# SonyCSLParis/audio-metrics

Measured on AMD Instinct MI355X. Metric: evaluate() embeddings/sec (FAD+KD+PRDC), 2×100k CLAP-512 sets, 1/2/4/8 GPUs, higher is better.
Workload: dtype f32

## Files before the change

audio-metrics_amd/csrc/pairwise.hip:

```cpp
#include "pairwise_common.h"
#include <algorithm>
#include <vector>
#include <cmath>
#include <type_traits>

namespace am {

__global__ void __launch_bounds__(256) row_sqnorm_kernel(const float* __restrict__ X, int64_t N, int64_t ld,
                                                         int D, float* __restrict__ out) {
    const int lane = threadIdx.x & 63;
    const int64_t row = (int64_t)blockIdx.x * 4 + (threadIdx.x >> 6);
    if (row >= N) return;
    const float* x = X + row * ld;
    float acc = 0.f;
    for (int k = lane * 4; k < D; k += 256) {
        const f32x4 v = load_k4(x, k, D);
        acc = fmaf(v.x, v.x, acc);
        acc = fmaf(v.y, v.y, acc);
        acc = fmaf(v.z, v.z, acc);
        acc = fmaf(v.w, v.w, acc);
    }
#pragma unroll
    for (int off = 32; off >= 1; off >>= 1) acc = acc + __shfl_xor(acc, off);
    if (lane == 0) out[row] = acc;
}

__device__ __forceinline__ float threshold_of_radius(float R) {
    if (!(R > 0.f)) return 0.f;
    if (isinf(R)) return R;
    float c = R * R;
    for (int it = 0; it < 8; ++it) {
        const float p = __uint_as_float(__float_as_uint(c) - 1u);
        if (c > 0.f && sqrt_rn(p) >= R) c = p; else break;
    }
    for (int it = 0; it < 8; ++it) {
        if (sqrt_rn(c) < R) c = __uint_as_float(__float_as_uint(c) + 1u); else break;
    }
    return c;
}

__global__ void threshold_kernel(const float* __restrict__ R, int64_t n, float* __restrict__ T) {
    const int64_t i = (int64_t)blockIdx.x * blockDim.x + threadIdx.x;
    if (i < n) T[i] = threshold_of_radius(R[i]);
}

struct DenseRows {
    const float* base;
    int64_t ld, n, tile0;
    __device__ __forceinline__ const float* operator()(int t, int row) const {
        const int64_t g = (tile0 + t) * TB + row;
        return g < n ? base + g * ld : nullptr;
    }
};

static inline int64_t cross_grouped_blocks(int64_t row_blocks, int nchunks, int grp_rows) {
    const int grp_chunks = 64 / grp_rows;
    const int64_t groups = ceil_div(row_blocks, grp_rows) * ceil_div(nchunks, grp_chunks);
// ... 1211 lines not shown
    hipLaunchKernelGGL(narrow64_kernel, dim3((unsigned)ceil_div(Nr, 256)), dim3(256), 0, st, rt, Nr, L.rt);
    hipLaunchKernelGGL(narrow64_kernel, dim3((unsigned)ceil_div(Nc, 256)), dim3(256), 0, st, ct, Nc, L.ct);
    hipLaunchKernelGGL(fill_u32_kernel, dim3((unsigned)ceil_div(Nr, 256)), dim3(256), 0, st, L.rmin, Nr, 0x7f800000u);
    AM_LAUNCH_CHECK();
    int rc;
    if ((rc = norms_of(nullptr, L.r32, Nr, L.ld32, D, L.rn, st)) != AM_OK) return rc;
    if ((rc = norms_of(nullptr, L.c32, Nc, L.ld32, D, L.cn, st)) != AM_OK) return rc;
    const Prdc64Hook h{R, C, ldr, ldc, rt, ct};
    if ((rc = run_cross_fast(L.r32, Nr, L.ld32, L.rn, L.rt, L.c32, Nc, L.ld32, L.cn, L.ct, D, L.plan, L.buf, col_count, L.rmin, row_any,
                             row_cover, false, st, nullptr, nullptr, &h)) != AM_OK)
        return rc;
    *fail_flag = L.buf.ov_count + 1;
    return AM_OK;
}

}

extern "C" int am_knn_radii_f32(const float* X, int64_t N, int64_t ldx, const float* Y, int64_t M, int64_t ldy,
                                int D, int k, float* out_r, void* ws, size_t ws_bytes, am_stream_t stream) {
    return knn_radii_impl(X, N, ldx, Y, M, ldy, D, k, out_r, ws, ws_bytes, stream, nullptr);
}

static bool prepared_ok(const am_prepared_set* p) { return p != nullptr && p->norms != nullptr && p->stats != nullptr && p->half != nullptr; }
static PreparedSet prepared_of(const am_prepared_set* p) { return PreparedSet{p->norms, p->stats, p->half}; }

extern "C" int64_t am_prepared_half_ld(int D) { return D < 1 ? 0 : half_ld(D); }

extern "C" int am_prepare_set_f32(const float* X, int64_t N, int64_t ld, int D, float* norms, uint32_t* stats4, uint16_t* half,
                                  am_stream_t stream) {
    int rc;
    if ((rc = check_matrix(X, N, ld, D, "X")) != AM_OK) return rc;
    AM_REQUIRE(norms && stats4 && half, AM_ERR_BAD_ARG, "null output pointer");
    hipStream_t st = static_cast<hipStream_t>(stream);
    if ((rc = launch_norms(X, N, ld, D, norms, st)) != AM_OK) return rc;
    AM_HIP_TRY(hipMemsetAsync(stats4, 0, 4 * sizeof(unsigned), st));
    return launch_to_half(X, N, ld, D, norms, stats4, 0, half, st);
}

extern "C" int am_knn_radii_prepared_f32(const float* X, int64_t N, int64_t ldx, int D, const am_prepared_set* prepared, int k,
                                         float* out_r, void* ws, size_t ws_bytes, am_stream_t stream) {
    AM_REQUIRE(prepared_ok(prepared), AM_ERR_BAD_ARG, "prepared set has a null member");
    const PreparedSet ps = prepared_of(prepared);
    return knn_radii_impl(X, N, ldx, X, N, ldx, D, k, out_r, ws, ws_bytes, stream, &ps);
}

extern "C" int am_filter_stats_enable(int64_t* device_slots) {
    if (device_slots == nullptr) {
        g_filter_stats = nullptr;
        g_filter_stats_device = -1;
        return AM_OK;
    }
    int dev = -1;
    AM_HIP_TRY(hipGetDevice(&dev));
    g_filter_stats = reinterpret_cast<long long*>(device_slots);
    g_filter_stats_device = dev;
    return AM_OK;
}

extern "C" int am_knn_path(int64_t N, int64_t M, int D, int k, int self) {
    if (N < 1 || M < 1 || D < 1 || k < 1) return -1;
    if (k > AM_MAX_K) return 4;
    const KnnPlan p = plan_knn(N, M, D, k, self != 0 && N == M);
    return !p.sym ? 0 : (knn_fast_enabled(N, D) ? (p.tile_rows == 256 ? 3 : 2) : 1);
}
extern "C" int am_prdc_path(int64_t Nr, int64_t Nc, int D) {
    if (Nr < 1 || Nc < 1 || D < 1) return -1;
    if (!cross_fast_enabled(Nr, Nc, D)) return 0;
    return plan_cross_fast(Nr, Nc, D).wide ? 3 : 2;
}
// ... 333 lines not shown
```

audio-metrics_amd/csrc/pairwise_fast.h:

```cpp
#pragma once

namespace am {

constexpr int EV_FAST = EV_DEFAULT | EV_F16 | EV_LDS;
constexpr int FAST_MAX_DIM = 4096;
constexpr int FAST_MIN_DIM = 1;
constexpr int FAST_DROP_BITS = 0;
static inline int half_drop_bits() {
    static const int n = std::min(std::max(env_int("AM_HALF_DROP_BITS", FAST_DROP_BITS), 0), 6);
    return n;
}
static inline float fast_c(int D) {
    const int n = half_drop_bits();
    const float rest = 1.9073486328125e-06f + 2.98023223876953125e-08f * sqrtf((float)D) + (float)(D + 1) * 4.76837158203125e-07f;
    if (n == 0) return 0.0009765625f + rest;
    const float u = ldexpf(1.f, -(11 - n)) + ldexpf(1.f, -11);
    return 2.f * u + u * u + rest;
}
constexpr int FAST_LDH_ALIGN = 64;

static inline int64_t half_ld(int D) { return (int64_t)(D + FAST_LDH_ALIGN - 1) / FAST_LDH_ALIGN * FAST_LDH_ALIGN; }

__global__ void __launch_bounds__(256) maxabs_bits_kernel(const float* __restrict__ X, int64_t N, int64_t ld, int D,
                                                          unsigned* __restrict__ out) {
// ... 56 lines not shown
static long long* g_filter_stats = nullptr;
static int g_filter_stats_device = -1;

static long long* filter_stats_for_current_device() {
    if (g_filter_stats == nullptr) return nullptr;
    int dev = -1;
    if (hipGetDevice(&dev) != hipSuccess || dev != g_filter_stats_device) return nullptr;
    return g_filter_stats;
}

__global__ void __launch_bounds__(256) filter_stats_kernel(const int* __restrict__ wgq_count, int64_t nwg, long long* __restrict__ stats,
                                                           int slot_calls, int slot_queued, const unsigned long long* spill64,
                                                           const int* spill32, int spill_cap, int slot_spill, const int* extra_a,
                                                           int slot_a, const int* extra_b, int slot_b) {
    long long q = 0;
    for (int64_t i = threadIdx.x; i < nwg; i += 256) q += wgq_count[i];
#pragma unroll
    for (int off = 32; off >= 1; off >>= 1) q += __shfl_xor(q, off);
    __shared__ long long red[4];
    if ((threadIdx.x & 63) == 0) red[threadIdx.x >> 6] = q;
    __syncthreads();
    if (threadIdx.x == 0) {
        long long spill = 0;
        if (spill64 != nullptr) spill = (long long)min(*spill64, (unsigned long long)spill_cap);
        if (spill32 != nullptr) spill = min(*spill32, spill_cap);
        atomicAdd(reinterpret_cast<unsigned long long*>(stats + slot_calls), 1ull);
        atomicAdd(reinterpret_cast<unsigned long long*>(stats + slot_queued), (unsigned long long)(red[0] + red[1] + red[2] + red[3] + spill));
        atomicAdd(reinterpret_cast<unsigned long long*>(stats + slot_spill), (unsigned long long)spill);
        if (extra_a != nullptr) atomicAdd(reinterpret_cast<unsigned long long*>(stats + slot_a), (unsigned long long)*extra_a);
        if (extra_b != nullptr) atomicAdd(reinterpret_cast<unsigned long long*>(stats + slot_b), (unsigned long long)*extra_b);
    }
}

static int launch_to_half(const float* X, int64_t N, int64_t ld, int D, const float* norms, unsigned* stats, int which,
                          uint16_t* Xh, hipStream_t st) {
    const int64_t ldh = half_ld(D);
    hipLaunchKernelGGL(max_bits_kernel, dim3(256), dim3(256), 0, st, norms, N, stats + which);
    hipLaunchKernelGGL(maxabs_bits_kernel, dim3((unsigned)std::min<int64_t>(ceil_div(N, 4), 1024)), dim3(256), 0, st, X, N, ld, D,
                       stats + 2 + which);
    const int64_t threads = N * (ldh / 8);
    hipLaunchKernelGGL(to_half_kernel, dim3((unsigned)ceil_div(threads, 256)), dim3(256), 0, st, X, N, ld, D, ldh,
                       stats + 2 + which, Xh, half_drop_bits());
    AM_LAUNCH_CHECK();
    return AM_OK;
}

struct PreparedSet {
    const float* norms;
    const unsigned* stats;
    const uint16_t* half;
};

__global__ void prepared_stats_kernel(const unsigned* __restrict__ stats, unsigned* __restrict__ maxn, int slot_norm, int slot_abs,
                                      int slot_abs2) {
    if (threadIdx.x == 0) {
        maxn[slot_norm] = stats[0];
        maxn[slot_abs] = stats[2];
        if (slot_abs2 >= 0) maxn[slot_abs2] = stats[2];
    }
}

static int norms_of(const PreparedSet* prep, const float* X, int64_t N, int64_t ld, int D, float* out, hipStream_t st) {
    if (prep != nullptr) {
        AM_HIP_TRY(hipMemcpyAsync(out, prep->norms, (size_t)N * sizeof(float), hipMemcpyDeviceToDevice, st));
        return AM_OK;
    }
    return launch_norms(X, N, ld, D, out, st);
}

__device__ __forceinline__ float exact_pair_dot(const float* __restrict__ xs, const float* __restrict__ y, int D) {
    float acc = 0.f;
    const int dp = (D + 7) / 8 * 8;
    for (int c = 0; c < dp; c += 8) {
        const f32x4 y0 = load_k4(y, c, D), y1 = load_k4(y, c + 4, D);
        const f32x4 x0 = *reinterpret_cast<const f32x4*>(xs + c), x1 = *reinterpret_cast<const f32x4*>(xs + c + 4);
#pragma unroll
        for (int s = 0; s < 4; ++s) {
            acc = fmaf(y0[s], x0[s], acc);
            acc = fmaf(y1[s], x1[s], acc);
        }
    }
    return acc;
}

constexpr int FAST_AUX_FLOATS = 6 * TB;
constexpr size_t FAST_LDS_BYTES = (ENGINE_LDS_FLOATS + FAST_AUX_FLOATS) * sizeof(float) + 16;

struct CrossFastEpilogue {
    const float* qnorm;
    const float* qthr;
    int64_t nq;
    float fc;
// ... 519 lines not shown
};

static CrossFastBuffers carve_cross_fast(Carver& c, int64_t Nr, int64_t Nc, int D, const CrossFastPlan& p) {
    CrossFastBuffers b;
    b.rb = c.take<uint16_t>((size_t)Nr * half_ld(D));
    b.cb = c.take<uint16_t>((size_t)Nc * half_ld(D));
    b.maxn = c.take<unsigned>(4);
    b.rmin_approx = c.take<unsigned>(Nr);
    b.wgq = c.take<uint2>((size_t)p.blocks * p.qcap);
    b.ovq = c.take<uint2>((size_t)p.ovcap);
    b.items = c.take<uint2>((size_t)p.blocks * ((p.qcap + 63) / 64));
    b.wgq_count = c.take<int>(p.blocks);
    b.ov_count = c.take<int>(4);
    return b;
}

static bool cross_fast_enabled(int64_t Nr, int64_t Nc, int D) {
    static const int on = env_int("AM_PRDC_FAST", 1);
    static const int min_pairs_env = env_int("AM_FAST_MIN_PAIRS_LOG2", 0);
    const int64_t min_pairs_n = min_pairs_env > 0 ? ((int64_t)1 << min_pairs_env)
                                                  : (D >= 256 ? (int64_t)1 << 24 : D >= 128 ? (int64_t)1 << 26 : D >= 32 ? (int64_t)100000000 : (int64_t)1 << 28);
    const size_t verify_lds = (size_t)(4 * ((D + 7) / 8 * 8) + 2048) * sizeof(float);
    return on != 0 && D >= FAST_MIN_DIM && D <= FAST_MAX_DIM && verify_lds <= 60 * 1024 && Nr * Nc >= min_pairs_n &&
           Nr < ((int64_t)1 << 31) && Nc < ((int64_t)1 << 31);
}

static int run_cross_fast(const float* R, int64_t Nr, int64_t ldr, const float* rn, const float* rt, const float* C, int64_t Nc,
                          int64_t ldc, const float* cn, const float* ct, int D, const CrossFastPlan& p, const CrossFastBuffers& b,
                          int32_t* col_count, unsigned* rmin, unsigned* rany, unsigned* rcov, bool want_min, hipStream_t st,
                          const PreparedSet* prep_r = nullptr, const PreparedSet* prep_c = nullptr, const Prdc64Hook* h64 = nullptr) {
    int rc;
    const float fc = h64 != nullptr ? fast_c(D) + 3.814697265625e-06f : fast_c(D);
    AM_REQUIRE(h64 == nullptr || (p.wide && !want_min), AM_ERR_BAD_ARG, "the float64 route is the 256-row form without row minima");
    AM_HIP_TRY(hipMemsetAsync(b.maxn, 0, 4 * sizeof(unsigned), st));
    AM_HIP_TRY(hipMemsetAsync(b.ov_count, 0, 4 * sizeof(int), st));
    if (prep_r != nullptr) hipLaunchKernelGGL(prepared_stats_kernel, dim3(1), dim3(64), 0, st, prep_r->stats, b.maxn, 0, 2, -1);
    else if ((rc = launch_to_half(R, Nr, ldr, D, rn, b.maxn, 0, b.rb, st)) != AM_OK) return rc;
    if (prep_c != nullptr) hipLaunchKernelGGL(prepared_stats_kernel, dim3(1), dim3(64), 0, st, prep_c->stats, b.maxn, 1, 3, -1);
    else if ((rc = launch_to_half(C, Nc, ldc, D, cn, b.maxn, 1, b.cb, st)) != AM_OK) return rc;
    hipLaunchKernelGGL(fill_u32_kernel, dim3((unsigned)ceil_div(Nr, 256)), dim3(256), 0, st, b.rmin_approx, Nr, 0x7f800000u);
    AM_LAUNCH_CHECK();
    const int64_t ldb = half_ld(D);
    const int Dh = (int)(ldb / 2);
    const float* Rb = reinterpret_cast<const float*>(prep_r != nullptr ? prep_r->half : b.rb);
    const float* Cb = reinterpret_cast<const float*>(prep_c != nullptr ? prep_c->half : b.cb);
    int* fail = b.ov_count + 1;
    {
        const void* kernels[] = {reinterpret_cast<const void*>(&cross_fast_kernel<true, true>),
                                 reinterpret_cast<const void*>(&cross_fast_kernel<true, false>),
                                 reinterpret_cast<const void*>(&cross_fast_kernel<false, true>),
                                 reinterpret_cast<const void*>(&cross_fast_kernel<false, false>)};
        for (const void* k : kernels)
            AM_HIP_TRY(ensure_dynamic_lds(k, (int)FAST_LDS_BYTES));
    }
    const int dbg = env_int("AM_FAST_DBG", 0);
    auto launch_filter = [&](auto kernel, unsigned grid, int nchunks, int qstride, int grp_rows) {
        hipLaunchKernelGGL(kernel, dim3(grid), dim3(ENGINE_THREADS), FAST_LDS_BYTES, st, Rb, Nr, ldb / 2, rn, rt, Cb, Nc, ldb / 2,
                           cn, ct, Dh, nchunks, qstride, b.maxn, b.rmin_approx, rany, rcov, col_count, b.wgq, p.qcap, b.wgq_count,
                           b.ovq, b.ov_count, p.ovcap, fail, dbg, fc, grp_rows);
    };
    const unsigned pre_grid = (unsigned)(ceil_div(Nr, TB) * p.pre_chunks);
    static const int pre_any = env_int("AM_FAST_PRE_ANY", 1);
    if (want_min) launch_filter(&cross_fast_kernel<true, true>, pre_grid, p.pre_chunks, p.qstride, 0);
    else if (pre_any == 1 && p.wide) {
        const int64_t samples = ceil_div(ceil_div(Nc, WIDE_TILE_ROWS), p.qstride), rbs = ceil_div(Nr, WIDE_TILE_ROWS);
        int chunks = 1;
        int64_t best_cost = INT64_MAX;
        for (int c = 1; c <= 12 && c <= samples; ++c) {
            const int64_t cost = ceil_div(rbs * c, 256) * (ceil_div(samples, c) + 1);
            if (cost < best_cost) {
                best_cost = cost;
                chunks = c;
            }
// ... 162 lines not shown
                for (int s = 0; s < KCAP; ++s)
                    if (v[s] > -INFINITY) list_insert<KCAP>(m, v[s]);
            }
            float* out = partial + ((int64_t)sw.W * N + i) * KCAP;
#pragma unroll
            for (int s = 0; s < KCAP; ++s) __hip_atomic_store(out + s, m[s], __ATOMIC_RELAXED, __HIP_MEMORY_SCOPE_AGENT);
            const float kthv = m[KCAP - 1];
            const float bound = kthv + 2.f * fc * (xnorm[i] + nmax);
            if (epi_row_in_sweep(thr, i)) atomicMin(reinterpret_cast<unsigned*>(thr) + i, __float_as_uint(bound));
        }
    }
}

__global__ void __launch_bounds__(256) knn_fast_bound_kernel(const float* __restrict__ in, float* __restrict__ thr,
                                                             const float* __restrict__ xnorm, int64_t n,
                                                             const unsigned* __restrict__ maxn, float factor ) {
    const int64_t i = (int64_t)blockIdx.x * 256 + threadIdx.x;
    if (i < n) thr[i] = in[i] + factor * (xnorm[i] + __uint_as_float(maxn[0]));
}

__device__ __forceinline__ void knn_file_approx(float* __restrict__ fval, unsigned* __restrict__ fidx, int* __restrict__ cnt,
                                                int cap, int64_t row, float v, unsigned partner) {
    const int slot = atomicAdd(cnt + row, 1);
    if (slot < cap) {
        fval[row * (int64_t)cap + slot] = v;
        fidx[row * (int64_t)cap + slot] = partner;
    }
}

__global__ void __launch_bounds__(256) knn_fast_scatter_kernel(const uint2* __restrict__ wgq, const float* __restrict__ wgv,
                                                               int qcap, int wcap, int nsub, const int* __restrict__ wgq_count,
                                                               float* __restrict__ fval, unsigned* __restrict__ fidx,
                                                               int* __restrict__ cnt, int cap, const float* __restrict__ thr,
                                                               const int* __restrict__ skip) {
    if (skip != nullptr && *skip != 0) return;
    const int n = wgq_count[blockIdx.x];
    const int64_t base = (int64_t)(blockIdx.x / (nsub + 1)) * qcap + (int64_t)(blockIdx.x % (nsub + 1)) * wcap;
    const uint2* q = wgq + base;
    const float* v = wgv + base;
    for (int e = threadIdx.x; e < n; e += 256) {
        const uint2 p = q[e];
        const unsigned a = p.x & ~FAST_BOTH;
        const float val = v[e];
        if (val <= thr[a]) knn_file_approx(fval, fidx, cnt, cap, a, val, p.y);
        if ((p.x & FAST_BOTH) && val <= thr[p.y]) knn_file_approx(fval, fidx, cnt, cap, p.y, val, a);
    }
}

__global__ void __launch_bounds__(256) knn_fast_scatter_spill_kernel(const uint2* __restrict__ ovq, const float* __restrict__ ovv,
                                                                     const unsigned long long* __restrict__ ovn, int ovcap,
                                                                     float* __restrict__ fval, unsigned* __restrict__ fidx,
                                                                     int* __restrict__ cnt, int cap, const float* __restrict__ thr,
                                                                     const int* __restrict__ skip) {
    if (skip != nullptr && *skip != 0) return;
    const int n = (int)min(*ovn, (unsigned long long)ovcap);
    for (int e = blockIdx.x * 256 + threadIdx.x; e < n; e += gridDim.x * 256) {
        const uint2 p = ovq[e];
        const unsigned a = p.x & ~FAST_BOTH;
        const float val = ovv[e];
        if (val <= thr[a]) knn_file_approx(fval, fidx, cnt, cap, a, val, p.y);
        if ((p.x & FAST_BOTH) && val <= thr[p.y]) knn_file_approx(fval, fidx, cnt, cap, p.y, val, a);
    }
}

template <int KCAP>
__global__ void __launch_bounds__(256) knn_fast_prune_kernel(const float* __restrict__ fval, const unsigned* __restrict__ fidx,
                                                             const int* __restrict__ cnt, int cap, int64_t N, int k1,
                                                             const float* __restrict__ xnorm, const unsigned* __restrict__ maxn,
                                                             uint2* __restrict__ pairs, float* __restrict__ pair_val, int pair_cap,
                                                             int* __restrict__ pair_count, int* __restrict__ cnt2, int partitioned,
                                                             float fc, int* __restrict__ gate, int* __restrict__ pair_start = nullptr,
                                                             int* __restrict__ pair_n = nullptr) {
    if (gate != nullptr && gate[0] != 0) return;
    const int64_t i = (int64_t)blockIdx.x * 256 + threadIdx.x;
    const int lane = threadIdx.x & 63;
    const int c = i < N ? cnt[i] : 0;
    const bool bad = i < N && (c > cap || (c < k1 && !partitioned));
    if (gate != nullptr) {
        const unsigned long long nb = __ballot(bad);
        if (lane == 0 && nb != 0ull) atomicAdd(gate + 3, __popcll(nb));
    }
    const float* fv = fval + i * (int64_t)cap;
    int ns = 0;
    float thr = -INFINITY;
    if (i < N && !bad) {
        float m[KCAP];
#pragma unroll
        for (int s = 0; s < KCAP; ++s) m[s] = INFINITY;
        for (int s = 0; s < c; ++s) {
            const float v = fmaxf(fv[s], 0.f);
            if (v < m[KCAP - 1]) list_insert<KCAP>(m, v);
        }
// ... 252 lines not shown
    }
    if (bound_slots != nullptr) {
#pragma unroll
        for (int off = 32; off >= 1; off >>= 1) {
            worst = fmaxf(worst, __shfl_xor(worst, off));
            measured += __shfl_xor(measured, off);
        }
        if (lane == 0 && measured != 0ull) {
            atomicMax(bound_slots, (unsigned long long)__float_as_uint(worst));
            atomicAdd(bound_slots + 1, measured);
        }
    }
}

template <int KCAP>
static int run_knn_fixup(const float* X, int64_t N, int64_t ld, const float* xn, int D, int k1, const int* ov_list, const int* ov_count,
                         const KnnFixup& x, float* out_r, hipStream_t st) {
    int rc;
    const int fcap = (int)x.capacity;
    const int64_t ldr = (D + 3) / 4 * 4;
    launch_knn_fixup<KCAP>(X, N, ld, xn, D, k1, ov_list, ov_count, out_r, KNN_FIX_BATCH_FROM, fcap, x.partial, st);
    hipLaunchKernelGGL(knn_gather_rows_kernel, dim3(1024), dim3(256), 0, st, X, ld, D, xn, ov_list, ov_count, KNN_FIX_BATCH_FROM, fcap,
                       x.rows, ldr, x.norms);
    AM_LAUNCH_CHECK();
    if ((rc = launch_knn<KCAP>(x.rows, fcap, ldr, x.norms, X, N, ld, xn, D, k1, choose_chunks(fcap, N), 1, false, x.partial, x.radii,
                               st, nullptr, ov_count, KNN_FIX_BATCH_FROM)) != AM_OK)
        return rc;
    hipLaunchKernelGGL(knn_scatter_radii_kernel, dim3(64), dim3(256), 0, st, x.radii, ov_list, ov_count, KNN_FIX_BATCH_FROM, fcap, out_r);
    AM_LAUNCH_CHECK();
    return AM_OK;
}

template <int KCAP>
__global__ void __launch_bounds__(256) knn_fast_predict_kernel(const float* __restrict__ partial, int64_t N, int nchunks, int k1,
                                                               const float* __restrict__ xnorm, const unsigned* __restrict__ maxn,
                                                               float fc, int* __restrict__ gate, unsigned char* __restrict__ flat_rows) {
    const int64_t i = (int64_t)blockIdx.x * 256 + threadIdx.x;
    bool flat = false;
    if (i < N) {
        float m[KCAP];
#pragma unroll
        for (int s = 0; s < KCAP; ++s) m[s] = partial[i * KCAP + s];
        for (int c = 1; c < nchunks; ++c) {
            const float* src = partial + ((int64_t)c * N + i) * KCAP;
            for (int s = 0; s < KCAP; ++s) list_insert<KCAP>(m, src[s]);
        }
        (void)k1;
        const float band = 2.f * fc * (xnorm[i] + __uint_as_float(maxn[0]));
        flat = m[KCAP - 1] < INFINITY && m[KCAP - 1] - m[1] <= band;
        if (i < N) flat_rows[i] = (flat && m[KCAP - 1] - m[1] <= 0.0625f * band) ? 1 : 0;
    }
    const unsigned long long b = __ballot(flat);
    if ((threadIdx.x & 63) == 0 && b != 0ull) atomicAdd(gate + 2, __popcll(b));
}

__global__ void __launch_bounds__(256) knn_fast_mask_flat_kernel(const unsigned char* __restrict__ flat_rows, const int* __restrict__ gate,
                                                                 float* __restrict__ thr, int* __restrict__ cnt, int64_t N) {
    if (gate[0] != 0) return;
    const int64_t i = (int64_t)blockIdx.x * 256 + threadIdx.x;
    if (i < N && flat_rows[i]) {
        thr[i] = -INFINITY;
        cnt[i] = FAST_ROW_OVERFLOW;
    }
}

__global__ void knn_fast_decide_kernel(int* __restrict__ gate, int64_t N, int k1, int stage, const int* __restrict__ pair_count,
                                       const unsigned* __restrict__ maxn, int* __restrict__ ov_count) {
    if (threadIdx.x != 0 || blockIdx.x != 0) return;
    if (stage == 0) {
        gate[0] = (int64_t)gate[2] * 8 > N ? 1 : 0;
    } else if (stage == 1) {
        const int64_t per_row = N / 160 > (int64_t)(8 * k1 + 16) ? N / 160 : (int64_t)(8 * k1 + 16);
        const bool volume = (int64_t)*pair_count > N * per_row;
        const bool fixups = (int64_t)gate[3] * 8 > N;
        gate[1] = (gate[0] != 0 || volume || fixups || !half_scale_ok(maxn[2])) ? 1 : 0;
    } else if (gate[1] != 0) {
        *ov_count = (int)(N < 0x7fffffff ? N : 0x7fffffff);
    }
}

static bool knn_fast_enabled(int64_t N, int D) {
    static const int on = env_int("AM_KNN_FAST", 1);
    static const int min_rows_env = env_int("AM_KNN_FAST_MIN_ROWS", 0);
    const int64_t min_rows = min_rows_env > 0 ? min_rows_env : (D >= 256 ? 6144 : D >= 128 ? 8192 : D >= 32 ? 12000 : 16384);
    return on != 0 && N >= min_rows && D >= FAST_MIN_DIM && D <= FAST_MAX_DIM && N < ((int64_t)1 << 31);
}

struct KnnFastBuffers {
    uint16_t* xb;
    unsigned* maxn;
    float* wgv;
    unsigned* fidx;
    int *cnt2, *pair_count;
    uint2* ovq;
    float* ovv;
    unsigned long long* ovn;
    int* gate;
    float* xpartial;
    unsigned char* flat_rows;
    KnnFixup fix;
};
constexpr int KNN_FAST_OVCAP = 1 << 22;

static KnnFastBuffers carve_knn_fast(Carver& c, int64_t N, int D, const KnnPlan& p) {
    KnnFastBuffers f;
    f.xb = c.take<uint16_t>((size_t)N * half_ld(D));
    f.maxn = c.take<unsigned>(4);
    f.wgv = c.take<float>((size_t)p.nwg * p.qcap);
    f.fidx = c.take<unsigned>((size_t)N * p.cap);
    f.cnt2 = c.take<int>(N + 2);
    f.pair_count = f.cnt2 ? f.cnt2 + N : nullptr;
// ... 6 lines not shown
    f.fix = carve_knn_fixup(c, N, D, p.kcap);
    return f;
}

static int wide_sample_chunks(int64_t row_blocks, int64_t samples) {
    int chunks = 1;
    int64_t best_cost = INT64_MAX;
    for (int c = 1; c <= 8 && c <= samples; ++c) {
        const int64_t cost = ceil_div(row_blocks * c, 256) * ceil_div(samples, c);
        if (cost < best_cost) {
            best_cost = cost;
            chunks = c;
        }
    }
    return chunks;
}

template <int KCAP>
static int run_knn_fast(const float* X, int64_t N, int64_t ld, int D, int k1, const KnnPlan& p, const KnnBuffers& b,
                        const KnnFastBuffers& f, float* out_r, hipStream_t st, int part = 0, int nparts = 1,
                        const float* bounds_in = nullptr, float* out_lists = nullptr, const PreparedSet* prep = nullptr,
                        const Knn64Hook* h64 = nullptr) {
    int rc;
    const float fc = h64 != nullptr ? fast_c(D) + 1.9073486328125e-06f : fast_c(D);
    const int64_t ldh = half_ld(D) / 2;
    const int Dh = (int)ldh;
    const float* Xb = reinterpret_cast<const float*>(prep != nullptr ? prep->half : f.xb);
    unsigned* maxn = f.maxn;
    float* thr = b.thr;
    static const int gate_on = env_int("AM_KNN_FAST_GATE", 1);
    int* gate = (gate_on != 0 && bounds_in == nullptr && out_lists == nullptr) ? f.gate : nullptr;
    const int* skip_sweep = gate;
    const int* skip_verify = gate != nullptr ? gate + 1 : nullptr;
    if (gate != nullptr) AM_HIP_TRY(hipMemsetAsync(gate, 0, 4 * sizeof(int), st));
    AM_HIP_TRY(hipMemsetAsync(maxn, 0, 4 * sizeof(unsigned), st));
    if (prep != nullptr) {
        hipLaunchKernelGGL(prepared_stats_kernel, dim3(1), dim3(64), 0, st, prep->stats, maxn, 0, 2, 3);
    } else {
        if ((rc = launch_to_half(X, N, ld, D, b.xn, maxn, 0, f.xb, st)) != AM_OK) return rc;
        AM_HIP_TRY(hipMemcpyAsync(maxn + 3, maxn + 2, sizeof(unsigned), hipMemcpyDeviceToDevice, st));
    }
    if (bounds_in != nullptr) {
        hipLaunchKernelGGL(knn_fast_bound_kernel, dim3((unsigned)ceil_div(N, 256)), dim3(256), 0, st, bounds_in, thr, b.xn, N, maxn, fc);
        AM_LAUNCH_CHECK();
    } else {
        int sample_chunks = p.pre_chunks;
        if (p.tile_rows == WIDE_TILE_ROWS) {
            const int64_t rb = ceil_div(N, WIDE_TILE_ROWS), samples = ceil_div(rb, p.pre_stride);
            sample_chunks = wide_sample_chunks(rb, samples);
            if ((rc = launch_knn_wide_sample(KCAP, Xb, N, ldh, b.xn, Dh, p.pre_stride, sample_chunks, maxn, b.partial, 0, N, st)) != AM_OK)
                return rc;
        } else if ((rc = launch_knn_vt<KCAP, EV_FAST, false>(Xb, N, ldh, b.xn, Xb, N, ldh, b.xn, Dh, p.pre_chunks, p.pre_stride,
                                                             b.partial, st, maxn)) != AM_OK) {
            return rc;
        }
        hipLaunchKernelGGL(knn_merge_kernel<KCAP>, dim3((unsigned)ceil_div(N, 256)), dim3(256), 0, st, b.partial, N, sample_chunks,
                           k1, 1, thr, static_cast<const int*>(nullptr));
        if (gate != nullptr) {
            hipLaunchKernelGGL(knn_fast_predict_kernel<KCAP>, dim3((unsigned)ceil_div(N, 256)), dim3(256), 0, st, b.partial, N,
                               sample_chunks, k1, b.xn, maxn, fc, gate, f.flat_rows);
            hipLaunchKernelGGL(knn_fast_decide_kernel, dim3(1), dim3(64), 0, st, gate, N, k1, 0, f.pair_count, maxn, b.ov_count);
        }
        hipLaunchKernelGGL(knn_fast_bound_kernel, dim3((unsigned)ceil_div(N, 256)), dim3(256), 0, st, thr, thr, b.xn, N, maxn, 2.f * fc);
        AM_LAUNCH_CHECK();
    }
    AM_HIP_TRY(hipMemsetAsync(b.cnt, 0, (size_t)(N + 1) * sizeof(int), st));
    AM_HIP_TRY(hipMemsetAsync(f.cnt2, 0, (size_t)(N + 2) * sizeof(int), st));
    if (gate != nullptr) {
        hipLaunchKernelGGL(knn_fast_mask_flat_kernel, dim3((unsigned)ceil_div(N, 256)), dim3(256), 0, st, f.flat_rows, gate, thr, b.cnt, N);
        AM_LAUNCH_CHECK();
    }
    AM_HIP_TRY(hipMemsetAsync(f.ovn, 0, sizeof(unsigned long long), st));
    const unsigned nwg = (unsigned)p.nwg;
    const int64_t nlist = (int64_t)p.nwin * N * KCAP;
    hipLaunchKernelGGL(fill_u32_kernel, dim3((unsigned)ceil_div(nlist, 256)), dim3(256), 0, st,
                       reinterpret_cast<unsigned*>(b.partial), nlist, 0x7f800000u);
    AM_LAUNCH_CHECK();
    {
        AM_HIP_TRY(ensure_dynamic_lds(reinterpret_cast<const void*>(&knn_fast_kernel<KCAP>), (int)PAIRWISE_LDS_BYTES + 16));
    }
    int qcap = p.qcap;
    const int nsub = p.tile_rows == WIDE_TILE_ROWS ? 8 : 4;
    unsigned nregions = nwg;
    int* region_counter = nullptr;
    if (nparts > 1) {
        const int64_t active = std::max<int64_t>(1, sym_active_items(ceil_div(N, p.tile_rows), p.win_tiles, p.nwin, p.per_win, part, nparts));
        const int64_t grown = std::min<int64_t>((int64_t)nwg * qcap / active, 1 << 18) / 16 * 16;
        qcap = (int)std::max<int64_t>(grown, qcap);
        nregions = (unsigned)std::min<int64_t>(active, (int64_t)nwg * p.qcap / qcap);
        region_counter = f.gate + 4;
        AM_HIP_TRY(hipMemsetAsync(region_counter, 0, sizeof(int), st));
        AM_HIP_TRY(hipMemsetAsync(b.wgq_count, 0, (size_t)nregions * (nsub + 1) * sizeof(int), st));
    }
    const int wcap = qcap / (2 * nsub);
    const unsigned nreg = nregions * (unsigned)(nsub + 1);
    static const int ovcap = std::max(0, std::min(env_int("AM_KNN_FAST_OVCAP", KNN_FAST_OVCAP), KNN_FAST_OVCAP));
    clock_begin(AM_KERNEL_KNN, st);
    if (p.tile_rows == WIDE_TILE_ROWS) {
        const auto launch_sweep = wide_stationary(Dh) ? &launch_knn_pstat : &launch_knn_wide;
        if ((rc = launch_sweep(KCAP, nwg, Xb, N, ldh, b.xn, thr, Dh, p.win_tiles, p.nwin, p.per_win, k1, maxn, b.partial, b.cnt,
                                  p.cap, b.wgq, f.wgv, qcap, b.wgq_count, part, nparts, fc, f.ovq, f.ovv, f.ovn, ovcap,
                                  skip_sweep, region_counter, st)) != AM_OK)
            return rc;
    } else {
        hipLaunchKernelGGL(knn_fast_kernel<KCAP>, dim3(nwg), dim3(ENGINE_THREADS), PAIRWISE_LDS_BYTES + 16, st, Xb, N, ldh, b.xn,
                           thr, Dh, p.win_tiles, p.nwin, p.per_win, k1, maxn, b.partial, b.cnt, p.cap, b.wgq, f.wgv, qcap,
                           b.wgq_count, part, nparts, fc, f.ovq, f.ovv, f.ovn, ovcap, skip_sweep, region_counter);
    }
    clock_end(AM_KERNEL_KNN, st);
    AM_LAUNCH_CHECK();
    hipLaunchKernelGGL(knn_fast_scatter_kernel, dim3(nreg), dim3(256), 0, st, b.wgq, f.wgv, qcap, wcap, nsub, b.wgq_count, b.cand,
                       f.fidx, b.cnt, p.cap, thr, skip_sweep);
    hipLaunchKernelGGL(knn_fast_scatter_spill_kernel, dim3(256), dim3(256), 0, st, f.ovq, f.ovv, f.ovn, ovcap, b.cand, f.fidx,
                       b.cnt, p.cap, thr, skip_sweep);
    AM_LAUNCH_CHECK();
    const int64_t pair_cap64 = std::min<int64_t>((int64_t)nwg * p.qcap, (int64_t)1 << 30);
    const int pair_cap = (int)pair_cap64;
    hipLaunchKernelGGL(knn_fast_prune_kernel<KCAP>, dim3((unsigned)ceil_div(N, 256)), dim3(256), 0, st, b.cand, f.fidx, b.cnt, p.cap,
                       N, k1, b.xn, maxn, b.wgq, f.wgv, pair_cap, f.pair_count, f.cnt2, out_lists != nullptr ? 1 : 0, fc, gate,
                       h64 != nullptr ? h64->pair_start : nullptr, h64 != nullptr ? h64->pair_n : nullptr);
    if (gate != nullptr)
        hipLaunchKernelGGL(knn_fast_decide_kernel, dim3(1), dim3(64), 0, st, gate, N, k1, 1, f.pair_count, maxn, b.ov_count);
    AM_LAUNCH_CHECK();
    if (h64 != nullptr) {
        AM_REQUIRE(gate != nullptr && out_lists == nullptr, AM_ERR_BAD_ARG, "the float64 route is the single-GPU form");
        clock_begin(AM_KERNEL_KNN_VERIFY, st);
        long long* stats64 = filter_stats_for_current_device();
        hipLaunchKernelGGL(knn_fast_select64_kernel, dim3((unsigned)ceil_div(N, 4 * KNN64_ROWS_PER_WAVE)), dim3(256), 0, st, h64->X, h64->ld, D, b.wgq,
                           h64->pair_start, h64->pair_n, N, k1, maxn, h64->out_r, gate, (const float*)f.wgv, (const float*)b.xn, fc,
                           stats64 != nullptr ? reinterpret_cast<unsigned long long*>(stats64) + 9 : nullptr);
        clock_end(AM_KERNEL_KNN_VERIFY, st);
        AM_LAUNCH_CHECK();
        if ((rc = knn64_self_gated(h64->X, N, h64->ld, D, h64->k, h64->out_r, h64->gen_ws, h64->gen_ws_bytes, gate + 1, st)) != AM_OK) return rc;
        hipLaunchKernelGGL(knn_fast_decide_kernel, dim3(1), dim3(64), 0, st, gate, N, k1, 2, f.pair_count, maxn, b.ov_count);
        AM_LAUNCH_CHECK();
        if (long long* stats = filter_stats_for_current_device()) {
            hipLaunchKernelGGL(filter_stats_kernel, dim3(1), dim3(256), 0, st, b.wgq_count, (int64_t)nreg, stats, 0, 1,
                               (const unsigned long long*)f.ovn, (const int*)nullptr, ovcap, 2, (const int*)f.pair_count, 3,
                               (const int*)b.ov_count, 4);
            AM_LAUNCH_CHECK();
        }
        return AM_OK;
    }
    clock_begin(AM_KERNEL_KNN_VERIFY, st);
    {
        AM_HIP_TRY(ensure_dynamic_lds(reinterpret_cast<const void*>(&knn_fast_verify_kernel), (int)VERIFY_LDS_BYTES));
    }
// ... 53 lines not shown
```

Baseline: 8.841 million.

## Fuse kNN setup, prepare, merge-predict and scatter kernels to cut launches

Merges several small kernels and memsets into fewer launches. Row norms and max-abs stats are computed in one prepare pass. Merge and predict are folded together, with a last-block gate decision replacing the separate decide kernel. Threshold, count, list and queue initialisation move into one setup kernel, and the spill scatter joins the main scatter. The aim is less launch and memset overhead and fewer passes over the data, at the cost of a more complex grid-wide last-block atomic protocol in which gate slot 5 must start at zero.

After: 8.833 million (median of 2 runs). No clear change (-0.1%).

```diff
diff --git a/audio-metrics_amd/csrc/pairwise.hip b/audio-metrics_amd/csrc/pairwise.hip
--- a/audio-metrics_amd/csrc/pairwise.hip
+++ b/audio-metrics_amd/csrc/pairwise.hip
@@ -6,12 +6,8 @@
 
 namespace am {
 
-__global__ void __launch_bounds__(256) row_sqnorm_kernel(const float* __restrict__ X, int64_t N, int64_t ld,
-                                                         int D, float* __restrict__ out) {
-    const int lane = threadIdx.x & 63;
-    const int64_t row = (int64_t)blockIdx.x * 4 + (threadIdx.x >> 6);
-    if (row >= N) return;
-    const float* x = X + row * ld;
+template <bool ABSMAX>
+__device__ __forceinline__ float wave_row_sqnorm(const float* __restrict__ x, int D, int lane, unsigned& absmax) {
     float acc = 0.f;
     for (int k = lane * 4; k < D; k += 256) {
         const f32x4 v = load_k4(x, k, D);
@@ -19,10 +15,48 @@
         acc = fmaf(v.y, v.y, acc);
         acc = fmaf(v.z, v.z, acc);
         acc = fmaf(v.w, v.w, acc);
+        if (ABSMAX) {
+            absmax = max(max(absmax, __float_as_uint(v.x) & 0x7fffffffu), __float_as_uint(v.y) & 0x7fffffffu);
+            absmax = max(max(absmax, __float_as_uint(v.z) & 0x7fffffffu), __float_as_uint(v.w) & 0x7fffffffu);
+        }
     }
 #pragma unroll
     for (int off = 32; off >= 1; off >>= 1) acc = acc + __shfl_xor(acc, off);
+    return acc;
+}
+
+__global__ void __launch_bounds__(256) row_sqnorm_kernel(const float* __restrict__ X, int64_t N, int64_t ld,
+                                                         int D, float* __restrict__ out) {
+    const int lane = threadIdx.x & 63;
+    const int64_t row = (int64_t)blockIdx.x * 4 + (threadIdx.x >> 6);
+    if (row >= N) return;
+    unsigned unused = 0u;
+    const float acc = wave_row_sqnorm<false>(X + row * ld, D, lane, unused);
     if (lane == 0) out[row] = acc;
+}
+
+__global__ void __launch_bounds__(256) prepare_rows_kernel(const float* __restrict__ X, int64_t N, int64_t ld, int D,
+                                                           float* __restrict__ out, unsigned* __restrict__ stats) {
+    const int lane = threadIdx.x & 63;
+    unsigned mabs = 0u, mnorm = 0u;
+    for (int64_t row = (int64_t)blockIdx.x * 4 + (threadIdx.x >> 6); row < N; row += (int64_t)gridDim.x * 4) {
+        const float acc = wave_row_sqnorm<true>(X + row * ld, D, lane, mabs);
+        if (lane == 0) out[row] = acc;
+        mnorm = max(mnorm, __float_as_uint(acc));
+    }
+#pragma unroll
+    for (int off = 32; off >= 1; off >>= 1) mabs = max(mabs, (unsigned)__shfl_xor((int)mabs, off));
+    __shared__ unsigned wave_max[2][4];
+    if (lane == 0) {
+        wave_max[0][threadIdx.x >> 6] = mnorm;
+        wave_max[1][threadIdx.x >> 6] = mabs;
+    }
+    __syncthreads();
+    if (threadIdx.x < 2) {
+        const unsigned* w = wave_max[threadIdx.x];
+        const unsigned m = max(max(w[0], w[1]), max(w[2], w[3]));
+        if (m != 0u) atomicMax(stats + 2 * threadIdx.x, m);
+    }
 }
 
 __device__ __forceinline__ float threshold_of_radius(float R) {
@@ -1300,9 +1334,11 @@
     if ((rc = check_matrix(X, N, ld, D, "X")) != AM_OK) return rc;
     AM_REQUIRE(norms && stats4 && half, AM_ERR_BAD_ARG, "null output pointer");
     hipStream_t st = static_cast<hipStream_t>(stream);
-    if ((rc = launch_norms(X, N, ld, D, norms, st)) != AM_OK) return rc;
     AM_HIP_TRY(hipMemsetAsync(stats4, 0, 4 * sizeof(unsigned), st));
-    return launch_to_half(X, N, ld, D, norms, stats4, 0, half, st);
+    hipLaunchKernelGGL(prepare_rows_kernel, dim3((unsigned)std::min<int64_t>(ceil_div(N, 4), 2048)), dim3(256), 0, st, X, N, ld, D,
+                       norms, stats4);
+    AM_LAUNCH_CHECK();
+    return launch_half_copy(X, N, ld, D, stats4 + 2, half, st);
 }
 
 extern "C" int am_knn_radii_prepared_f32(const float* X, int64_t N, int64_t ldx, int D, const am_prepared_set* prepared, int k,
diff --git a/audio-metrics_amd/csrc/pairwise_fast.h b/audio-metrics_amd/csrc/pairwise_fast.h
--- a/audio-metrics_amd/csrc/pairwise_fast.h
+++ b/audio-metrics_amd/csrc/pairwise_fast.h
@@ -112,17 +112,21 @@
     }
 }
 
+static int launch_half_copy(const float* X, int64_t N, int64_t ld, int D, const unsigned* maxabs_bits, uint16_t* Xh, hipStream_t st) {
+    const int64_t ldh = half_ld(D);
+    const int64_t threads = N * (ldh / 8);
+    hipLaunchKernelGGL(to_half_kernel, dim3((unsigned)ceil_div(threads, 256)), dim3(256), 0, st, X, N, ld, D, ldh, maxabs_bits, Xh,
+                       half_drop_bits());
+    AM_LAUNCH_CHECK();
+    return AM_OK;
+}
+
 static int launch_to_half(const float* X, int64_t N, int64_t ld, int D, const float* norms, unsigned* stats, int which,
                           uint16_t* Xh, hipStream_t st) {
-    const int64_t ldh = half_ld(D);
     hipLaunchKernelGGL(max_bits_kernel, dim3(256), dim3(256), 0, st, norms, N, stats + which);
     hipLaunchKernelGGL(maxabs_bits_kernel, dim3((unsigned)std::min<int64_t>(ceil_div(N, 4), 1024)), dim3(256), 0, st, X, N, ld, D,
                        stats + 2 + which);
-    const int64_t threads = N * (ldh / 8);
-    hipLaunchKernelGGL(to_half_kernel, dim3((unsigned)ceil_div(threads, 256)), dim3(256), 0, st, X, N, ld, D, ldh,
-                       stats + 2 + which, Xh, half_drop_bits());
-    AM_LAUNCH_CHECK();
-    return AM_OK;
+    return launch_half_copy(X, N, ld, D, stats + 2 + which, Xh, st);
 }
 
 struct PreparedSet {
@@ -138,6 +142,17 @@
         maxn[slot_abs] = stats[2];
         if (slot_abs2 >= 0) maxn[slot_abs2] = stats[2];
     }
+}
+
+__global__ void __launch_bounds__(256) cross_fast_head_kernel(const unsigned* __restrict__ stats_r, const unsigned* __restrict__ stats_c,
+                                                              unsigned* __restrict__ maxn, int* __restrict__ ov_count,
+                                                              unsigned* __restrict__ rmin_approx, int64_t Nr) {
+    if (blockIdx.x == 0 && threadIdx.x < 4) {
+        const int t = threadIdx.x;
+        maxn[t] = ((t & 1) ? stats_c : stats_r)[t & 2];
+        ov_count[t] = 0;
+    }
+    for (int64_t i = (int64_t)blockIdx.x * 256 + threadIdx.x; i < Nr; i += (int64_t)gridDim.x * 256) rmin_approx[i] = 0x7f800000u;
 }
 
 static int norms_of(const PreparedSet* prep, const float* X, int64_t N, int64_t ld, int D, float* out, hipStream_t st) {
@@ -723,13 +738,18 @@
     int rc;
     const float fc = h64 != nullptr ? fast_c(D) + 3.814697265625e-06f : fast_c(D);
     AM_REQUIRE(h64 == nullptr || (p.wide && !want_min), AM_ERR_BAD_ARG, "the float64 route is the 256-row form without row minima");
-    AM_HIP_TRY(hipMemsetAsync(b.maxn, 0, 4 * sizeof(unsigned), st));
-    AM_HIP_TRY(hipMemsetAsync(b.ov_count, 0, 4 * sizeof(int), st));
-    if (prep_r != nullptr) hipLaunchKernelGGL(prepared_stats_kernel, dim3(1), dim3(64), 0, st, prep_r->stats, b.maxn, 0, 2, -1);
-    else if ((rc = launch_to_half(R, Nr, ldr, D, rn, b.maxn, 0, b.rb, st)) != AM_OK) return rc;
-    if (prep_c != nullptr) hipLaunchKernelGGL(prepared_stats_kernel, dim3(1), dim3(64), 0, st, prep_c->stats, b.maxn, 1, 3, -1);
-    else if ((rc = launch_to_half(C, Nc, ldc, D, cn, b.maxn, 1, b.cb, st)) != AM_OK) return rc;
-    hipLaunchKernelGGL(fill_u32_kernel, dim3((unsigned)ceil_div(Nr, 256)), dim3(256), 0, st, b.rmin_approx, Nr, 0x7f800000u);
+    if (prep_r != nullptr && prep_c != nullptr) {
+        hipLaunchKernelGGL(cross_fast_head_kernel, dim3((unsigned)std::min<int64_t>(ceil_div(Nr, 256), 1024)), dim3(256), 0, st,
+                           prep_r->stats, prep_c->stats, b.maxn, b.ov_count, b.rmin_approx, Nr);
+    } else {
+        AM_HIP_TRY(hipMemsetAsync(b.maxn, 0, 4 * sizeof(unsigned), st));
+        AM_HIP_TRY(hipMemsetAsync(b.ov_count, 0, 4 * sizeof(int), st));
+        if (prep_r != nullptr) hipLaunchKernelGGL(prepared_stats_kernel, dim3(1), dim3(64), 0, st, prep_r->stats, b.maxn, 0, 2, -1);
+        else if ((rc = launch_to_half(R, Nr, ldr, D, rn, b.maxn, 0, b.rb, st)) != AM_OK) return rc;
+        if (prep_c != nullptr) hipLaunchKernelGGL(prepared_stats_kernel, dim3(1), dim3(64), 0, st, prep_c->stats, b.maxn, 1, 3, -1);
+        else if ((rc = launch_to_half(C, Nc, ldc, D, cn, b.maxn, 1, b.cb, st)) != AM_OK) return rc;
+        hipLaunchKernelGGL(fill_u32_kernel, dim3((unsigned)ceil_div(Nr, 256)), dim3(256), 0, st, b.rmin_approx, Nr, 0x7f800000u);
+    }
     AM_LAUNCH_CHECK();
     const int64_t ldb = half_ld(D);
     const int Dh = (int)(ldb / 2);
@@ -958,8 +978,22 @@
                                                                int qcap, int wcap, int nsub, const int* __restrict__ wgq_count,
                                                                float* __restrict__ fval, unsigned* __restrict__ fidx,
                                                                int* __restrict__ cnt, int cap, const float* __restrict__ thr,
-                                                               const int* __restrict__ skip) {
+                                                               const int* __restrict__ skip, unsigned nreg,
+                                                               const uint2* __restrict__ ovq, const float* __restrict__ ovv,
+                                                               const unsigned long long* __restrict__ ovn, int ovcap) {
     if (skip != nullptr && *skip != 0) return;
+    if (blockIdx.x >= nreg) {
+        const int n = (int)min(*ovn, (unsigned long long)ovcap);
+        const int nspill = (int)(gridDim.x - nreg);
+        for (int e = (int)(blockIdx.x - nreg) * 256 + threadIdx.x; e < n; e += nspill * 256) {
+            const uint2 p = ovq[e];
+            const unsigned a = p.x & ~FAST_BOTH;
+            const float val = ovv[e];
+            if (val <= thr[a]) knn_file_approx(fval, fidx, cnt, cap, a, val, p.y);
+            if ((p.x & FAST_BOTH) && val <= thr[p.y]) knn_file_approx(fval, fidx, cnt, cap, p.y, val, a);
+        }
+        return;
+    }
     const int n = wgq_count[blockIdx.x];
     const int64_t base = (int64_t)(blockIdx.x / (nsub + 1)) * qcap + (int64_t)(blockIdx.x % (nsub + 1)) * wcap;
     const uint2* q = wgq + base;
@@ -968,22 +1002,6 @@
         const uint2 p = q[e];
         const unsigned a = p.x & ~FAST_BOTH;
         const float val = v[e];
-        if (val <= thr[a]) knn_file_approx(fval, fidx, cnt, cap, a, val, p.y);
-        if ((p.x & FAST_BOTH) && val <= thr[p.y]) knn_file_approx(fval, fidx, cnt, cap, p.y, val, a);
-    }
-}
-
-__global__ void __launch_bounds__(256) knn_fast_scatter_spill_kernel(const uint2* __restrict__ ovq, const float* __restrict__ ovv,
-                                                                     const unsigned long long* __restrict__ ovn, int ovcap,
-                                                                     float* __restrict__ fval, unsigned* __restrict__ fidx,
-                                                                     int* __restrict__ cnt, int cap, const float* __restrict__ thr,
-                                                                     const int* __restrict__ skip) {
-    if (skip != nullptr && *skip != 0) return;
-    const int n = (int)min(*ovn, (unsigned long long)ovcap);
-    for (int e = blockIdx.x * 256 + threadIdx.x; e < n; e += gridDim.x * 256) {
-        const uint2 p = ovq[e];
-        const unsigned a = p.x & ~FAST_BOTH;
-        const float val = ovv[e];
         if (val <= thr[a]) knn_file_approx(fval, fidx, cnt, cap, a, val, p.y);
         if ((p.x & FAST_BOTH) && val <= thr[p.y]) knn_file_approx(fval, fidx, cnt, cap, p.y, val, a);
     }
@@ -1302,9 +1320,10 @@
 }
 
 template <int KCAP>
-__global__ void __launch_bounds__(256) knn_fast_predict_kernel(const float* __restrict__ partial, int64_t N, int nchunks, int k1,
-                                                               const float* __restrict__ xnorm, const unsigned* __restrict__ maxn,
-                                                               float fc, int* __restrict__ gate, unsigned char* __restrict__ flat_rows) {
+__global__ void __launch_bounds__(256) knn_fast_merge_predict_kernel(const float* __restrict__ partial, int64_t N, int nchunks, int k1,
+                                                                     const float* __restrict__ xnorm, const unsigned* __restrict__ maxn,
+                                                                     float fc, int* __restrict__ gate, unsigned char* __restrict__ flat_rows,
+                                                                     float* __restrict__ thr) {
     const int64_t i = (int64_t)blockIdx.x * 256 + threadIdx.x;
     bool flat = false;
     if (i < N) {
@@ -1315,22 +1334,27 @@
             const float* src = partial + ((int64_t)c * N + i) * KCAP;
             for (int s = 0; s < KCAP; ++s) list_insert<KCAP>(m, src[s]);
         }
-        (void)k1;
+        float r2 = m[0];
+#pragma unroll
+        for (int s = 1; s < KCAP; ++s)
+            if (s == k1 - 1) r2 = m[s];
+        thr[i] = r2;
         const float band = 2.f * fc * (xnorm[i] + __uint_as_float(maxn[0]));
         flat = m[KCAP - 1] < INFINITY && m[KCAP - 1] - m[1] <= band;
-        if (i < N) flat_rows[i] = (flat && m[KCAP - 1] - m[1] <= 0.0625f * band) ? 1 : 0;
+        flat_rows[i] = (flat && m[KCAP - 1] - m[1] <= 0.0625f * band) ? 1 : 0;
     }
     const unsigned long long b = __ballot(flat);
     if ((threadIdx.x & 63) == 0 && b != 0ull) atomicAdd(gate + 2, __popcll(b));
-}
-
-__global__ void __launch_bounds__(256) knn_fast_mask_flat_kernel(const unsigned char* __restrict__ flat_rows, const int* __restrict__ gate,
-                                                                 float* __restrict__ thr, int* __restrict__ cnt, int64_t N) {
-    if (gate[0] != 0) return;
-    const int64_t i = (int64_t)blockIdx.x * 256 + threadIdx.x;
-    if (i < N && flat_rows[i]) {
-        thr[i] = -INFINITY;
-        cnt[i] = FAST_ROW_OVERFLOW;
+    __shared__ int last;
+    __threadfence();
+    __syncthreads();
+    if (threadIdx.x == 0) {
+        last = atomicAdd(gate + 5, 1) == (int)gridDim.x - 1;
+        if (last) {
+            __threadfence();
+            const int flat_total = atomicAdd(gate + 2, 0);
+            gate[0] = (int64_t)flat_total * 8 > N ? 1 : 0;
+        }
     }
 }
 
@@ -1347,6 +1371,54 @@
     } else if (gate[1] != 0) {
         *ov_count = (int)(N < 0x7fffffff ? N : 0x7fffffff);
     }
+}
+
+__global__ void knn_fast_head_kernel(const unsigned* __restrict__ stats, unsigned* __restrict__ maxn, int* __restrict__ gate) {
+    const int t = threadIdx.x;
+    if (t < 4) maxn[t] = t == 0 ? stats[0] : t == 1 ? 0u : stats[2];
+    if (gate != nullptr && t < 6 && t != 4) gate[t] = 0;
+}
+
+__global__ void __launch_bounds__(256) knn_fast_setup_kernel(const float* in, float* thr, const float* __restrict__ xnorm, int64_t N,
+                                                             const unsigned* __restrict__ maxn, float factor,
+                                                             const unsigned char* __restrict__ flat_rows, const int* __restrict__ gate,
+                                                             int* __restrict__ cnt, int* __restrict__ cnt2,
+                                                             unsigned long long* __restrict__ ovn, unsigned* __restrict__ lists,
+                                                             int64_t nlist, int* __restrict__ region_counter,
+                                                             int* __restrict__ wgq_count, int64_t nwgq) {
+    const int64_t t0 = (int64_t)blockIdx.x * 256 + threadIdx.x, stride = (int64_t)gridDim.x * 256;
+    const bool mask = gate != nullptr && gate[0] == 0;
+    const float nmax = __uint_as_float(maxn[0]);
+    for (int64_t i = t0; i < N + 2; i += stride) {
+        if (i < N) {
+            float bound = in[i] + factor * (xnorm[i] + nmax);
+            int c = 0;
+            if (mask && flat_rows[i]) {
+                bound = -INFINITY;
+                c = FAST_ROW_OVERFLOW;
+            }
+            thr[i] = bound;
+            cnt[i] = c;
+        } else if (i == N) {
+            cnt[N] = 0;
+        }
+        cnt2[i] = 0;
+    }
+    if (t0 == 0) {
+        *ovn = 0ull;
+        if (region_counter != nullptr) *region_counter = 0;
+    }
+    if (wgq_count != nullptr)
+        for (int64_t i = t0; i < nwgq; i += stride) wgq_count[i] = 0;
+    const unsigned v = 0x7f800000u;
+    const int64_t to_aligned = (int64_t)((16u - (unsigned)(reinterpret_cast<uintptr_t>(lists) & 15u)) & 15u) / 4;
+    const int64_t head = to_aligned < nlist ? to_aligned : nlist;
+    const int64_t nvec = (nlist - head) / 4;
+    uint4* body = reinterpret_cast<uint4*>(lists + head);
+    for (int64_t i = t0; i < nvec; i += stride) body[i] = make_uint4(v, v, v, v);
+    if (t0 < head) lists[t0] = v;
+    const int64_t tail = head + nvec * 4;
+    if (tail + t0 < nlist) lists[tail + t0] = v;
 }
 
 static bool knn_fast_enabled(int64_t N, int D) {
@@ -1419,18 +1491,17 @@
     int* gate = (gate_on != 0 && bounds_in == nullptr && out_lists == nullptr) ? f.gate : nullptr;
     const int* skip_sweep = gate;
     const int* skip_verify = gate != nullptr ? gate + 1 : nullptr;
-    if (gate != nullptr) AM_HIP_TRY(hipMemsetAsync(gate, 0, 4 * sizeof(int), st));
-    AM_HIP_TRY(hipMemsetAsync(maxn, 0, 4 * sizeof(unsigned), st));
     if (prep != nullptr) {
-        hipLaunchKernelGGL(prepared_stats_kernel, dim3(1), dim3(64), 0, st, prep->stats, maxn, 0, 2, 3);
+        hipLaunchKernelGGL(knn_fast_head_kernel, dim3(1), dim3(64), 0, st, prep->stats, maxn, gate);
     } else {
+        if (gate != nullptr) AM_HIP_TRY(hipMemsetAsync(gate, 0, 8 * sizeof(int), st));
+        AM_HIP_TRY(hipMemsetAsync(maxn, 0, 4 * sizeof(unsigned), st));
         if ((rc = launch_to_half(X, N, ld, D, b.xn, maxn, 0, f.xb, st)) != AM_OK) return rc;
         AM_HIP_TRY(hipMemcpyAsync(maxn + 3, maxn + 2, sizeof(unsigned), hipMemcpyDeviceToDevice, st));
     }
-    if (bounds_in != nullptr) {
-        hipLaunchKernelGGL(knn_fast_bound_kernel, dim3((unsigned)ceil_div(N, 256)), dim3(256), 0, st, bounds_in, thr, b.xn, N, maxn, fc);
-        AM_LAUNCH_CHECK();
-    } else {
+    const float* bound_in = bounds_in;
+    float bound_factor = fc;
+    if (bounds_in == nullptr) {
         int sample_chunks = p.pre_chunks;
         if (p.tile_rows == WIDE_TILE_ROWS) {
             const int64_t rb = ceil_div(N, WIDE_TILE_ROWS), samples = ceil_div(rb, p.pre_stride);
@@ -1441,28 +1512,19 @@
                                                              b.partial, st, maxn)) != AM_OK) {
             return rc;
         }
-        hipLaunchKernelGGL(knn_merge_kernel<KCAP>, dim3((unsigned)ceil_div(N, 256)), dim3(256), 0, st, b.partial, N, sample_chunks,
-                           k1, 1, thr, static_cast<const int*>(nullptr));
         if (gate != nullptr) {
-            hipLaunchKernelGGL(knn_fast_predict_kernel<KCAP>, dim3((unsigned)ceil_div(N, 256)), dim3(256), 0, st, b.partial, N,
-                               sample_chunks, k1, b.xn, maxn, fc, gate, f.flat_rows);
-            hipLaunchKernelGGL(knn_fast_decide_kernel, dim3(1), dim3(64), 0, st, gate, N, k1, 0, f.pair_count, maxn, b.ov_count);
-        }
-        hipLaunchKernelGGL(knn_fast_bound_kernel, dim3((unsigned)ceil_div(N, 256)), dim3(256), 0, st, thr, thr, b.xn, N, maxn, 2.f * fc);
+            hipLaunchKernelGGL(knn_fast_merge_predict_kernel<KCAP>, dim3((unsigned)ceil_div(N, 256)), dim3(256), 0, st, b.partial, N,
+                               sample_chunks, k1, b.xn, maxn, fc, gate, f.flat_rows, thr);
+        } else {
+            hipLaunchKernelGGL(knn_merge_kernel<KCAP>, dim3((unsigned)ceil_div(N, 256)), dim3(256), 0, st, b.partial, N, sample_chunks,
+                               k1, 1, thr, static_cast<const int*>(nullptr));
+        }
         AM_LAUNCH_CHECK();
-    }
-    AM_HIP_TRY(hipMemsetAsync(b.cnt, 0, (size_t)(N + 1) * sizeof(int), st));
-    AM_HIP_TRY(hipMemsetAsync(f.cnt2, 0, (size_t)(N + 2) * sizeof(int), st));
-    if (gate != nullptr) {
-        hipLaunchKernelGGL(knn_fast_mask_flat_kernel, dim3((unsigned)ceil_div(N, 256)), dim3(256), 0, st, f.flat_rows, gate, thr, b.cnt, N);
-        AM_LAUNCH_CHECK();
-    }
-    AM_HIP_TRY(hipMemsetAsync(f.ovn, 0, sizeof(unsigned long long), st));
+        bound_in = thr;
+        bound_factor = 2.f * fc;
+    }
     const unsigned nwg = (unsigned)p.nwg;
     const int64_t nlist = (int64_t)p.nwin * N * KCAP;
-    hipLaunchKernelGGL(fill_u32_kernel, dim3((unsigned)ceil_div(nlist, 256)), dim3(256), 0, st,
-                       reinterpret_cast<unsigned*>(b.partial), nlist, 0x7f800000u);
-    AM_LAUNCH_CHECK();
     {
         AM_HIP_TRY(ensure_dynamic_lds(reinterpret_cast<const void*>(&knn_fast_kernel<KCAP>), (int)PAIRWISE_LDS_BYTES + 16));
     }
@@ -1476,8 +1538,14 @@
         qcap = (int)std::max<int64_t>(grown, qcap);
         nregions = (unsigned)std::min<int64_t>(active, (int64_t)nwg * p.qcap / qcap);
         region_counter = f.gate + 4;
-        AM_HIP_TRY(hipMemsetAsync(region_counter, 0, sizeof(int), st));
-        AM_HIP_TRY(hipMemsetAsync(b.wgq_count, 0, (size_t)nregions * (nsub + 1) * sizeof(int), st));
+    }
+    {
+        const int64_t nwgq = nparts > 1 ? (int64_t)nregions * (nsub + 1) : 0;
+        const int64_t work = std::max<int64_t>({N + 2, nlist / 4, nwgq});
+        hipLaunchKernelGGL(knn_fast_setup_kernel, dim3((unsigned)std::min<int64_t>(ceil_div(work, 256), 2048)), dim3(256), 0, st, bound_in,
+                           thr, b.xn, N, maxn, bound_factor, f.flat_rows, static_cast<const int*>(gate), b.cnt, f.cnt2, f.ovn,
+                           reinterpret_cast<unsigned*>(b.partial), nlist, region_counter, nparts > 1 ? b.wgq_count : nullptr, nwgq);
+        AM_LAUNCH_CHECK();
     }
     const int wcap = qcap / (2 * nsub);
     const unsigned nreg = nregions * (unsigned)(nsub + 1);
@@ -1496,10 +1564,8 @@
     }
     clock_end(AM_KERNEL_KNN, st);
     AM_LAUNCH_CHECK();
-    hipLaunchKernelGGL(knn_fast_scatter_kernel, dim3(nreg), dim3(256), 0, st, b.wgq, f.wgv, qcap, wcap, nsub, b.wgq_count, b.cand,
-                       f.fidx, b.cnt, p.cap, thr, skip_sweep);
-    hipLaunchKernelGGL(knn_fast_scatter_spill_kernel, dim3(256), dim3(256), 0, st, f.ovq, f.ovv, f.ovn, ovcap, b.cand, f.fidx,
-                       b.cnt, p.cap, thr, skip_sweep);
+    hipLaunchKernelGGL(knn_fast_scatter_kernel, dim3(nreg + 256u), dim3(256), 0, st, b.wgq, f.wgv, qcap, wcap, nsub, b.wgq_count, b.cand,
+                       f.fidx, b.cnt, p.cap, thr, skip_sweep, nreg, f.ovq, f.ovv, f.ovn, ovcap);
     AM_LAUNCH_CHECK();
     const int64_t pair_cap64 = std::min<int64_t>((int64_t)nwg * p.qcap, (int64_t)1 << 30);
     const int pair_cap = (int)pair_cap64;
```
